# Don-Yin/VAE-GAN

Measured on NVIDIA B200. Metric: train_images_per_sec, higher is better.
Workload: dtype bf16

## Files before the change

### vae_gan_b200/csrc/conv_tc.cu

```cuda
#include <algorithm>
#include <array>
#include <map>
#include <mutex>
#include <vector>
#include "vg_common.cuh"
#include "sm100_ptx.cuh"

namespace vg {

struct TcTap {
  int8_t map, dy, dx, pad_;
  int32_t wrow;
};
struct TcPhase {
  int32_t ntaps, oy_off, ox_off, pad_;
  TcTap taps[16];
};
struct alignas(64) TcConvParams {
  CUtensorMap in_maps[4];
  CUtensorMap w_map;
  TcPhase phases[4];
  int tiles_x, tiles_y, tiles_n;
  int tw_log2, th_log2, TW, TH, TN;
  int gw, gh, gn;
  int k_chunks;
  int n_out;
  int n_store;
  int OH, OW, os;
  int out_f32;
  int ksplit, k_per_split;
  void* out;
  const float* bias;
  const float* colscale;
  const float* sigma;
  int sigma_group_n;
  float act_slope;
  const void* residual;
  void* out2;
  const float* post_scale;
  const float* post_shift;
  float post_slope;
  CUtensorMap out_maps[4];
  int tma_store;
  int* det_locks;
  long long det_split_stride;
};

struct alignas(64) TcWgradParams {
  CUtensorMap s_maps[4];
  CUtensorMap u_map;
  TcTap taps[16];
  int ntaps, cs_chunks, cs, cu;
  int tiles_x, tiles_y, tiles_n, TW, TH, TN;
  int n_boxes, boxes_per_split;
  int packed;
  float* dw;
  int* det_locks;
  long long det_split_stride;
};

constexpr int kTcThreads = 256;
constexpr int kABytes = 128 * 128;
constexpr int kStageBytes = 32 * 64;

template <int STAGES, int A_BYTES, int B_BYTES, int NACC, int EW>
struct TcSmem {
  static constexpr int kStages = STAGES, kA = A_BYTES, kB = B_BYTES;
  static constexpr int kBytes =
      1024 + STAGES * (A_BYTES + B_BYTES) + (2 * STAGES + NACC) * 8 + 16 + (EW > 0 ? 16 + 512 + EW * kStageBytes : 0);
  uint8_t* a;
  uint8_t* b;
  uint64_t* full;
  uint64_t* empty;
  uint64_t* acc;
  uint32_t* tmem_slot;
  uint8_t* stage;
  __device__ explicit TcSmem(uint8_t* raw) {
    a = raw + ((1024u - (ptx::smem_u32(raw) & 1023u)) & 1023u);
    b = a + STAGES * A_BYTES;
    full = reinterpret_cast<uint64_t*>(b + STAGES * B_BYTES);
    empty = full + STAGES;
    acc = empty + STAGES;
    tmem_slot = reinterpret_cast<uint32_t*>(acc + NACC);
    stage = reinterpret_cast<uint8_t*>((reinterpret_cast<uintptr_t>(tmem_slot + 4) + 511) & ~(uintptr_t)511);
  }
};

template <int BN, int STAGES>
using ConvSmem = TcSmem<STAGES, kABytes, BN * 128, 1, 4>;
template <int CTAS, int BN, int MT, int STAGES, int EW>
using ConvPersistSmem = TcSmem<STAGES, MT * kABytes, (BN / CTAS) * 128, 4, EW>;
template <int NB, int STAGES>
using WgradSmem = TcSmem<STAGES, (2 + NB) * 8192, 0, 1, 0>;

template <int CTAS, int TMEM_COLS, class Smem, class InitAcc>
__device__ __forceinline__ uint32_t tc_prologue(const Smem& sm, const CUtensorMap* map0, const CUtensorMap* map1, InitAcc init_acc) {
  const int warp = threadIdx.x >> 5, lane = threadIdx.x & 31;
  if (warp == 0 && lane == 0) {
    ptx::prefetch_tmap(map0);
    ptx::prefetch_tmap(map1);
  }
  if (warp == 1 && lane == 0) {
    for (int s = 0; s < Smem::kStages; ++s) {
      ptx::mbar_init(&sm.full[s], 1);
      ptx::mbar_init(&sm.empty[s], 1);
    }
    init_acc();
    ptx::fence_barrier_init();
  }
  if (warp == 2) {
    if constexpr (CTAS == 2) ptx::tmem_alloc_pair<TMEM_COLS>(sm.tmem_slot);
    else ptx::tmem_alloc<TMEM_COLS>(sm.tmem_slot);
  }
  ptx::tc_fence_before();
  if constexpr (CTAS == 2) ptx::cluster_sync();
  else __syncthreads();
  ptx::tc_fence_after();
  vg::pdl_entry();
  return *sm.tmem_slot;
}

template <int CTAS, int TMEM_COLS>
__device__ __forceinline__ void tc_teardown(uint32_t tmem_base) {
  ptx::tc_fence_before();
  if constexpr (CTAS == 2) ptx::cluster_sync();
  else __syncthreads();
  if ((threadIdx.x >> 5) == 2) {
    if constexpr (CTAS == 2) ptx::tmem_dealloc_pair<TMEM_COLS>(tmem_base);
    else ptx::tmem_dealloc<TMEM_COLS>(tmem_base);
  }
}

struct Tile { int x0, y0, n0; };
template <class P>
__device__ __forceinline__ Tile tile_origin(const P& p, int t) {
  const int tx = t % p.tiles_x; t /= p.tiles_x;
  const int ty = t % p.tiles_y;
  const int tn = t / p.tiles_y;
  return Tile{tx * p.TW, ty * p.TH, tn * p.TN};
}

template <class Smem>
struct RingPos {
  int stage = 0;
  uint32_t phase = 0;
  __device__ __forceinline__ bool next() {
    if (++stage < Smem::kStages) return false;
    stage = 0;
    phase ^= 1u;
    return true;
  }
};

template <bool INF>
__device__ __forceinline__ void epilogue_chunk(const TcConvParams& p, const uint32_t (&r)[32], bool valid, long long opix, int gn,
                                               int ncol, bool first_chunk, uint8_t* stage, int sx, int sy, int sn, int z) {
  const int lane = threadIdx.x & 31;
  const bool add_bias = p.ksplit <= 1 || z == 0;
  float v[32];
#pragma unroll
  for (int j = 0; j < 32; ++j) v[j] = __uint_as_float(r[j]);
  if (p.sigma != nullptr && valid) {
    const float inv = 1.0f / __ldg(p.sigma + (p.sigma_group_n > 0 ? gn / p.sigma_group_n : 0));
#pragma unroll
    for (int j = 0; j < 32; ++j) v[j] *= inv;
  }
  if (p.bias != nullptr && add_bias) {
#pragma unroll
    for (int j = 0; j < 32; ++j)
      if (ncol + j < p.n_out) v[j] += __ldg(p.bias + ncol + j);
  }
  if (p.colscale != nullptr && valid) {
    const float* cs = p.colscale + (long long)gn * p.n_out + ncol;
#pragma unroll
// ... 122 lines not shown
        }
        *reinterpret_cast<uint4*>(o + j) = make_uint4(w[0], w[1], w[2], w[3]);
      }
    }
  }
}


__device__ __forceinline__ const TcPhase& conv_slice(const TcConvParams& p, int z, int& kb0, int& kb1) {
  const TcPhase& ph = p.phases[p.ksplit > 1 ? 0 : z];
  const int total = ph.ntaps * p.k_chunks;
  if (p.ksplit > 1) { kb0 = z * p.k_per_split; kb1 = min(total, kb0 + p.k_per_split); }
  else { kb0 = 0; kb1 = total; }
  if (kb1 < kb0) kb1 = kb0;
  return ph;
}

template <int CTAS, int MT, class Smem>
__device__ __forceinline__ void load_item(const TcConvParams& p, const TcPhase& ph, int kb0, int kb1, const Tile (&t)[MT], int nvalid,
                                          int wrow0, uint32_t rank, const Smem& sm, RingPos<Smem>& pos) {
  int tp = kb0 / p.k_chunks, kc = kb0 % p.k_chunks;
  for (int i = kb0; i < kb1; ++i) {
    const TcTap tap = ph.taps[tp];
    const CUtensorMap* im = &p.in_maps[tap.map];
    ptx::mbar_wait(&sm.empty[pos.stage], pos.phase ^ 1u);
    if (ptx::elect_one()) {
      uint8_t* a = sm.a + pos.stage * Smem::kA;
      uint8_t* b = sm.b + pos.stage * Smem::kB;
      if constexpr (CTAS == 2) {
        if (rank == 0) ptx::mbar_arrive_expect_tx(&sm.full[pos.stage], 2 * (Smem::kA + Smem::kB));
        const uint32_t bar = ptx::mapa(ptx::smem_u32(&sm.full[pos.stage]), 0);
#pragma unroll
        for (int m = 0; m < MT; ++m)
          ptx::tma_load_4d_pair(a + m * kABytes, im, bar, kc * 64, t[m].x0 + tap.dx, t[m].y0 + tap.dy, t[m].n0);
        ptx::tma_load_2d_pair(b, &p.w_map, bar, kc * 64, tap.wrow + wrow0);
      } else {
        ptx::mbar_arrive_expect_tx(&sm.full[pos.stage], nvalid * kABytes + Smem::kB);
#pragma unroll
        for (int m = 0; m < MT; ++m)
          if (m < nvalid)
            ptx::tma_load_4d(a + m * kABytes, im, &sm.full[pos.stage], kc * 64, t[m].x0 + tap.dx, t[m].y0 + tap.dy, t[m].n0);
        ptx::tma_load_2d(b, &p.w_map, &sm.full[pos.stage], kc * 64, tap.wrow + wrow0);
      }
    }
    __syncwarp();
    pos.next();
    if (++kc == p.k_chunks) { kc = 0; ++tp; }
  }
}

template <int CTAS>
__device__ __forceinline__ void commit_to(uint64_t* bar) {
  if constexpr (CTAS == 2) ptx::mma_commit_pair(bar, 3);
  else ptx::mma_commit(bar);
}

template <int CTAS, int BN, int MT, class Smem>
__device__ __forceinline__ void mma_item(uint32_t acc, int num_k, int nvalid, const Smem& sm, RingPos<Smem>& pos, uint32_t a_lo0,
                                         uint32_t b_lo0, uint32_t& a_lo, uint32_t& b_lo) {
  constexpr uint32_t idesc = ptx::make_idesc_bf16(128 * CTAS, BN, 0, 0);
  constexpr uint32_t kDescHi = ptx::smem_desc_hi(1024);
  for (int i = 0; i < num_k; ++i) {
    ptx::mbar_wait(&sm.full[pos.stage], pos.phase);
    ptx::tc_fence_after();
    if (ptx::elect_one()) {
#pragma unroll
      for (int m = 0; m < MT; ++m) {
        if (m < nvalid) {
#pragma unroll
          for (int k = 0; k < 4; ++k) {
            const uint32_t d = acc + (uint32_t)(m * BN), a = a_lo + (uint32_t)((m * kABytes + k * 32) >> 4),
                           b = b_lo + (uint32_t)((k * 32) >> 4);
            if constexpr (CTAS == 2) ptx::mma_bf16_ss_pair_lohi(d, a, b, kDescHi, idesc, (i | k) != 0);
            else ptx::mma_bf16_ss_lohi(d, a, b, kDescHi, idesc, (i | k) != 0);
          }
        }
      }
      commit_to<CTAS>(&sm.empty[pos.stage]);
    }
    __syncwarp();
    if (pos.next()) { a_lo = a_lo0; b_lo = b_lo0; }
    else { a_lo += (uint32_t)(Smem::kA >> 4); b_lo += (uint32_t)(Smem::kB >> 4); }
  }
}

struct EpiWarp {
  int ew, q, cgrp;
  int xl, yl, nl;
  int xl0, yl0, nl0;
  __device__ explicit EpiWarp(const TcConvParams& p) {
    ew = (int)(threadIdx.x >> 5) - 4;
    q = ew & 3;
    cgrp = ew >> 2;
    const int row = q * 32 + (threadIdx.x & 31), row0 = q * 32;
    xl = row & (p.TW - 1);
    yl = (row >> p.tw_log2) & (p.TH - 1);
    nl = row >> (p.tw_log2 + p.th_log2);
    xl0 = row0 & (p.TW - 1), yl0 = (row0 >> p.tw_log2) & (p.TH - 1), nl0 = row0 >> (p.tw_log2 + p.th_log2);
  }
};

template <int BN, int EW, bool INF>
__device__ __forceinline__ void drain_tile(const TcConvParams& p, const TcPhase& ph, const EpiWarp& e, uint32_t acc, bool has_k, Tile t,
                                           bool live, int ncol0, int z, uint8_t* stage_base) {
  const int gx = t.x0 + e.xl, gy = t.y0 + e.yl, gn = t.n0 + e.nl;
  const bool valid = gx < p.gw && gy < p.gh && gn < p.gn && live;
  const long long opix = ((long long)gn * p.OH + (long long)gy * p.os + ph.oy_off) * p.OW + (long long)gx * p.os + ph.ox_off;
#pragma unroll(EW == 4 ? BN / 32 : 1)
  for (int i = 0; i < BN / EW / 8; ++i) {
    const int c = EW == 4 ? i : i * (EW / 4) + e.cgrp;
    const int c0 = c * 32;
    uint32_t r[32];
    if (has_k) {
      ptx::tmem_ld_32x32(acc + ((uint32_t)(e.q * 32) << 16) + (uint32_t)c0, r);
      ptx::tmem_ld_wait();
    } else {
#pragma unroll
      for (int j = 0; j < 32; ++j) r[j] = 0u;
    }
    epilogue_chunk<INF>(p, r, valid, opix, gn, ncol0 + c0, c == 0, stage_base + e.ew * kStageBytes, t.x0 + e.xl0, t.y0 + e.yl0,
                        t.n0 + e.nl0, z);
  }
}

template <int BN, int STAGES, bool INF>
__global__ void __launch_bounds__(kTcThreads) tc_conv_kernel(const __grid_constant__ TcConvParams p) {
  using Smem = ConvSmem<BN, STAGES>;
  extern __shared__ uint8_t smem_raw[];
  const Smem sm(smem_raw);
  uint64_t* const tmem_full = sm.acc;
  const int warp = threadIdx.x >> 5, lane = threadIdx.x & 31;
  const int z = (int)blockIdx.z;
  int kb0, kb1;
  const TcPhase& ph = conv_slice(p, z, kb0, kb1);
  const bool has_k = kb1 > kb0;
  const Tile t = tile_origin(p, (int)blockIdx.x);
  const int ncol0 = blockIdx.y * BN;
  const uint32_t tmem_base = tc_prologue<1, BN>(sm, &p.w_map, &p.in_maps[0], [&] { ptx::mbar_init(tmem_full, 1); });

  if (has_k) {
    RingPos<Smem> pos;
    if (warp == 0) {
      const Tile ts[1] = {t};
      load_item<1, 1>(p, ph, kb0, kb1, ts, 1, ncol0, 0, sm, pos);
    } else if (warp == 1) {
      const uint32_t a_lo0 = ptx::smem_desc_lo(ptx::smem_u32(sm.a), 16), b_lo0 = ptx::smem_desc_lo(ptx::smem_u32(sm.b), 16);
      uint32_t a_lo = a_lo0, b_lo = b_lo0;
      mma_item<1, BN, 1>(tmem_base, kb1 - kb0, 1, sm, pos, a_lo0, b_lo0, a_lo, b_lo);
      if (ptx::elect_one()) ptx::mma_commit(tmem_full);
      __syncwarp();
    }
  }

  if (warp >= 4) {
    if (has_k) {
      ptx::mbar_wait(tmem_full, 0);
      ptx::tc_fence_after();
    }
    int* const det_lock = (p.det_locks != nullptr && p.ksplit > 1) ? p.det_locks + (blockIdx.y * gridDim.x + blockIdx.x) : nullptr;
    if (det_lock) {
      if (lane == 0) det_wait_turn(det_lock, z);
      __syncwarp();
    }
    const bool live = !(p.ksplit > 1 && !has_k && p.det_split_stride == 0);
    drain_tile<BN, 4, INF>(p, ph, EpiWarp(p), tmem_base, has_k, t, live, ncol0, z, sm.stage);
    if (det_lock) {
      __threadfence();
      asm volatile("bar.sync 2, 128;" ::: "memory");
      if (warp == 4 && lane == 0) det_publish_turn(det_lock, z + 1 == p.ksplit ? 0 : z + 1);
    }
    if (!INF && p.tma_store && lane == 0) ptx::bulk_wait_group0();
  }
  tc_teardown<1, BN>(tmem_base);
}

template <int CTAS, int BN, int MT, int STAGES, int EW, bool INF>
__device__ __forceinline__ void conv_persistent(const TcConvParams& p, int n_ntiles, int n_groups, int n_work) {
  static_assert(EW == 4 || EW == 8, "4 or 8 epilogue warps");
  constexpr int kAccCols = MT * BN;
  constexpr int kTmemCols = 2 * kAccCols;
  static_assert(kTmemCols <= 512 && kTmemCols >= 32, "TMEM budget");
  using Smem = ConvPersistSmem<CTAS, BN, MT, STAGES, EW>;
  extern __shared__ uint8_t smem_raw[];
  const Smem sm(smem_raw);
  uint64_t* const acc_full = sm.acc;
  uint64_t* const acc_empty = sm.acc + 2;
  const int warp = threadIdx.x >> 5, lane = threadIdx.x & 31;
  const uint32_t rank = CTAS == 2 ? ptx::cluster_ctarank() : 0u;
  const int w_first = blockIdx.x / CTAS, w_step = gridDim.x / CTAS;
  const int total_tiles = p.tiles_x * p.tiles_y * p.tiles_n;
  const uint32_t tmem_base = tc_prologue<CTAS, kTmemCols>(sm, &p.w_map, &p.in_maps[0], [&] {
    for (int a = 0; a < 2; ++a) {
      ptx::mbar_init(&acc_full[a], 1);
      ptx::mbar_init(&acc_empty[a], CTAS * EW);
    }
  });

  auto decode = [&](int w, int& z, int& nt, int& g) {
    const int per_z = n_ntiles * n_groups;
    z = w / per_z;
    const int r = w - z * per_z;
    nt = r / n_groups;
    g = r - nt * n_groups;
  };
  auto tiles_of = [&](int g, int& tile0, int& nvalid) {
    tile0 = (g * CTAS + (int)rank) * MT;
    nvalid = CTAS == 2 ? MT : min(MT, total_tiles - tile0);
  };

  if (warp == 0) {
    RingPos<Smem> pos;
    for (int w = w_first; w < n_work; w += w_step) {
      int z, nt, g, kb0, kb1, tile0, nvalid;
      decode(w, z, nt, g);
      const TcPhase& ph = conv_slice(p, z, kb0, kb1);
      if (kb1 == kb0) continue;
      tiles_of(g, tile0, nvalid);
      Tile t[MT];
#pragma unroll
      for (int m = 0; m < MT; ++m) t[m] = tile_origin(p, tile0 + m);
      load_item<CTAS, MT>(p, ph, kb0, kb1, t, nvalid, nt * BN + (int)rank * (BN / CTAS), rank, sm, pos);
    }
  } else if (warp == 1) {
    if (rank == 0) {
      const uint32_t a_lo0 = ptx::smem_desc_lo(ptx::smem_u32(sm.a), 16), b_lo0 = ptx::smem_desc_lo(ptx::smem_u32(sm.b), 16);
      uint32_t a_lo = a_lo0, b_lo = b_lo0;
      RingPos<Smem> pos;
      int it = 0;
      for (int w = w_first; w < n_work; w += w_step) {
        int z, nt, g, kb0, kb1, tile0, nvalid;
        decode(w, z, nt, g);
        conv_slice(p, z, kb0, kb1);
        if (kb1 == kb0) continue;
        tiles_of(g, tile0, nvalid);
        const int as = it & 1;
        ptx::mbar_wait(&acc_empty[as], (uint32_t)(((it >> 1) & 1) ^ 1));
        ptx::tc_fence_after();
        mma_item<CTAS, BN, MT>(tmem_base + (uint32_t)(as * kAccCols), kb1 - kb0, nvalid, sm, pos, a_lo0, b_lo0, a_lo, b_lo);
        if (ptx::elect_one()) commit_to<CTAS>(&acc_full[as]);
        __syncwarp();
        ++it;
      }
    }
  } else if (warp >= 4) {
    const EpiWarp e(p);
    int it = 0;
    for (int w = w_first; w < n_work; w += w_step) {
      int z, nt, g, kb0, kb1, tile0, nvalid;
      decode(w, z, nt, g);
      const TcPhase& ph = conv_slice(p, z, kb0, kb1);
      const bool has_k = kb1 > kb0;
      if (!has_k && p.ksplit > 1) continue;
      tiles_of(g, tile0, nvalid);
      const int as = it & 1;
      if (has_k) {
        ptx::mbar_wait(&acc_full[as], (uint32_t)((it >> 1) & 1));
        ptx::tc_fence_after();
      }
#pragma unroll 1
      for (int m = 0; m < nvalid; ++m)
        drain_tile<BN, EW, INF>(p, ph, e, tmem_base + (uint32_t)(as * kAccCols + m * BN), has_k, tile_origin(p, tile0 + m), true, nt * BN,
                                z, sm.stage);
      if (has_k) {
        ptx::tc_fence_before();
        __syncwarp();
        if (lane == 0) {
          if constexpr (CTAS == 2) ptx::mbar_arrive_cluster(ptx::mapa(ptx::smem_u32(&acc_empty[as]), 0));
          else ptx::mbar_arrive(&acc_empty[as]);
        }
        ++it;
      }
    }
    if (!INF && p.tma_store && lane == 0) ptx::bulk_wait_group0();
  }
  tc_teardown<CTAS, kTmemCols>(tmem_base);
}

template <int BN, int MT, int STAGES, int EW, bool INF>
__global__ void __launch_bounds__(128 + 32 * EW, 1)
    tc_conv_persist_kernel(const __grid_constant__ TcConvParams p, int n_ntiles, int n_groups, int n_work) {
  conv_persistent<1, BN, MT, STAGES, EW, INF>(p, n_ntiles, n_groups, n_work);
}

template <int BN, int MT, int STAGES, int EW, bool INF>
__global__ void __cluster_dims__(2, 1, 1) __launch_bounds__(128 + 32 * EW, 1)
    tc_conv_pair_kernel(const __grid_constant__ TcConvParams p, int n_ntiles, int n_groups, int n_work) {
  conv_persistent<2, BN, MT, STAGES, EW, INF>(p, n_ntiles, n_groups, n_work);
}

template <int NB, int STAGES>
__global__ void __launch_bounds__(kTcThreads) tc_wgrad_kernel(const __grid_constant__ TcWgradParams p) {
  using Smem = WgradSmem<NB, STAGES>;
  extern __shared__ uint8_t smem_raw[];
  constexpr int BN = NB * 64;
  constexpr int kStageBytes = Smem::kA;
  const Smem sm(smem_raw);
  uint8_t* const smem = sm.a;
  uint64_t* const full = sm.full;
  uint64_t* const empty = sm.empty;
  uint64_t* const tmem_full = sm.acc;

  const int warp = threadIdx.x >> 5, lane = threadIdx.x & 31;
  const int n_slabs = p.ntaps * p.cs_chunks;
  const int slab0 = blockIdx.x * 2;
  const bool has2 = slab0 + 1 < n_slabs;
  const int slab1 = has2 ? slab0 + 1 : slab0;
  const int box_begin = blockIdx.z * p.boxes_per_split;
  const int box_end = min(p.n_boxes, box_begin + p.boxes_per_split);
  const int num_k = max(0, box_end - box_begin);

  const uint32_t tmem_base = tc_prologue<1, BN>(sm, &p.u_map, &p.s_maps[0], [&] { ptx::mbar_init(tmem_full, 1); });

  if (num_k > 0) {
    if (warp == 0) {
      const int tapA = slab0 / p.cs_chunks, chA = slab0 % p.cs_chunks;
      const int tapB = slab1 / p.cs_chunks, chB = slab1 % p.cs_chunks;
      const TcTap ta = p.taps[tapA], tb = p.taps[tapB];
      int stage = 0;
      uint32_t phase = 0;
      for (int b = box_begin; b < box_end; ++b) {
        const Tile t = tile_origin(p, b);
        const int x0 = t.x0, y0 = t.y0, n0 = t.n0;
        ptx::mbar_wait(&empty[stage], phase ^ 1u);
        if (ptx::elect_one()) {
          ptx::mbar_arrive_expect_tx(&full[stage], kStageBytes);
          uint8_t* st = smem + stage * kStageBytes;
          ptx::tma_load_4d(st, &p.s_maps[ta.map], &full[stage], chA * 64, x0 + ta.dx, y0 + ta.dy, n0);
          ptx::tma_load_4d(st + 8192, &p.s_maps[tb.map], &full[stage], chB * 64, x0 + tb.dx, y0 + tb.dy, n0);
#pragma unroll
          for (int j = 0; j < NB; ++j)
            ptx::tma_load_4d(st + (2 + j) * 8192, &p.u_map, &full[stage], (blockIdx.y * NB + j) * 64, x0, y0, n0);
        }
        __syncwarp();
        if (++stage == STAGES) { stage = 0; phase ^= 1u; }
      }
    } else if (warp == 1) {
      constexpr uint32_t idesc = ptx::make_idesc_bf16(128, BN, 1, 1);
      constexpr uint32_t kDescHi = ptx::smem_desc_hi(1024);
      const uint32_t a_lo0 = ptx::smem_desc_lo(ptx::smem_u32(smem), 8192);
      uint32_t a_lo = a_lo0;
      int stage = 0;
      uint32_t phase = 0;
      for (int i = 0; i < num_k; ++i) {
        ptx::mbar_wait(&full[stage], phase);
        ptx::tc_fence_after();
        if (ptx::elect_one()) {
#pragma unroll
          for (int k = 0; k < 4; ++k)
            ptx::mma_bf16_ss_lohi(tmem_base, a_lo + (uint32_t)((k * 2048) >> 4), a_lo + (uint32_t)((2 * 8192 + k * 2048) >> 4), kDescHi,
                                  idesc, (i | k) != 0);
          ptx::mma_commit(&empty[stage]);
        }
        __syncwarp();
        if (++stage == STAGES) { stage = 0; phase ^= 1u; a_lo = a_lo0; }
        else a_lo += (uint32_t)(kStageBytes >> 4);
      }
      if (ptx::elect_one()) ptx::mma_commit(tmem_full);
      __syncwarp();
    }
  }

  int* const det_lock = p.det_locks != nullptr ? p.det_locks + (blockIdx.y * gridDim.x + blockIdx.x) : nullptr;
  if (warp >= 4 && det_lock) {
    if (lane == 0) det_wait_turn(det_lock, (int)blockIdx.z);
    __syncwarp();
  }
  if (warp >= 4 && num_k > 0) {
    const int q = warp - 4;
    const int row = q * 32 + lane;
    const int slab = (row < 64) ? slab0 : slab1;
// ... 141 lines not shown
  int l = 0;
  while ((1 << l) < v) ++l;
  return l;
}

static void choose_box(int gw, int gh, int gn, int pixels, int* TW, int* TH, int* TN) {
  double best = 1e30;
  int bw = 1, bh = 1;
  for (int tw = 1; tw <= pixels; tw *= 2)
    for (int th = 1; tw * th <= pixels; th *= 2) {
      int tn = pixels / (tw * th);
      if (tw > 256 || th > 256 || tn > 256) continue;
      double padded = (double)cdiv(gw, tw) * tw * (double)cdiv(gh, th) * th * (double)cdiv(gn, tn) * tn;
      double score = padded - 1e-3 * tw - 1e-6 * th;
      if (score < best) { best = score; bw = tw; bh = th; }
    }
  *TW = bw; *TH = bh; *TN = pixels / (bw * bh);
}

static bool tc_common_supported(const VgConvDesc* d) {
  if (g_force_simt) return false;
  if (d->act_dtype != VG_BF16) return false;
  if (d->stride != 1 && d->stride != 2) return false;
  if (d->kh != d->kw || d->kh * d->kw > 16) return false;
  if (d->stride == 2 && ((d->transposed ? d->h_out : d->h_in) % 2 != 0 || (d->transposed ? d->w_out : d->w_in) % 2 != 0)) return false;
  return get_encode() != nullptr;
}

bool tc_conv_supported(const VgConvDesc* d, bool dgrad) {
  const int c_red = dgrad ? d->c_out : d->c_in;
  const int n_out = dgrad ? d->c_in : d->c_out;
  return c_red % 64 == 0 && (n_out % 64 == 0 || n_out == 1) && tc_common_supported(d);
}

bool tc_wgrad_supported(const VgConvDesc* d) {
  return d->c_in % 64 == 0 && d->c_out % 64 == 0 && tc_common_supported(d);
}

template <auto Kernel, class... Args>
static int launch(dim3 grid, int threads, int smem, cudaStream_t s, const Args&... args) {
  static std::once_flag once;
  static cudaError_t attr_err = cudaSuccess;
  std::call_once(once, [smem] { attr_err = cudaFuncSetAttribute(Kernel, cudaFuncAttributeMaxDynamicSharedMemorySize, smem); });
  VG_CUDA(attr_err);
  vg::Launch(grid, threads, smem, s)(Kernel, args...);
  VG_LAUNCHED();
  return VG_OK;
}

static void build_gather_taps(TcPhase* ph, int k, int stride, int pad, int n_out) {
  ph->ntaps = 0; ph->oy_off = 0; ph->ox_off = 0;
  for (int ky = 0; ky < k; ++ky)
    for (int kx = 0; kx < k; ++kx) {
      TcTap& t = ph->taps[ph->ntaps++];
      const int ty = ky - pad, tx = kx - pad;
      if (stride == 1) {
        t.map = 0; t.dy = (int8_t)ty; t.dx = (int8_t)tx;
      } else {
        const int py = ((ty % 2) + 2) % 2, px = ((tx % 2) + 2) % 2;
        t.map = (int8_t)(py * 2 + px);
        t.dy = (int8_t)((ty - py) / 2);
        t.dx = (int8_t)((tx - px) / 2);
      }
      t.pad_ = 0;
      t.wrow = (ky * k + kx) * n_out;
    }
}
static void build_scatter_phase(TcPhase* ph, int k, int stride, int pad, int n_out, int phy, int phx) {
  ph->ntaps = 0; ph->oy_off = phy; ph->ox_off = phx;
  for (int ky = 0; ky < k; ++ky) {
    if (((phy + pad - ky) % stride + stride) % stride != 0) continue;
    for (int kx = 0; kx < k; ++kx) {
      if (((phx + pad - kx) % stride + stride) % stride != 0) continue;
      TcTap& t = ph->taps[ph->ntaps++];
      t.map = 0;
      t.dy = (int8_t)((phy + pad - ky) / stride);
      t.dx = (int8_t)((phx + pad - kx) / stride);
      t.pad_ = 0;
      t.wrow = (ky * k + kx) * n_out;
    }
  }
}

enum TuneForm { kFormAuto = 0, kFormOneShot = 1, kFormPersist = 2, kFormPair = 3 };
using TuneKey = std::array<int, 10>;
struct TuneVal { int bn, form; };
static std::map<TuneKey, TuneVal> g_tune;
static std::vector<TuneKey> g_tune_seen;
static bool g_tune_record = false;
static std::mutex g_tune_mu;
static TuneKey tune_key(const VgConvDesc* d, bool dgrad) {
  return TuneKey{dgrad ? 1 : 0, d->n, d->h_in, d->w_in, d->c_in, d->c_out, d->kh, d->stride, d->pad, d->transposed ? 1 : 0};
}
static TuneVal tune_lookup(const VgConvDesc* d, bool dgrad) {
  std::lock_guard<std::mutex> lk(g_tune_mu);
  const TuneKey k = tune_key(d, dgrad);
  if (g_tune_record && std::find(g_tune_seen.begin(), g_tune_seen.end(), k) == g_tune_seen.end()) g_tune_seen.push_back(k);
  auto it = g_tune.find(k);
  return it == g_tune.end() ? TuneVal{0, kFormAuto} : it->second;
}
int tc_tune_set(const VgConvDesc* d, int dgrad, int bn, int form) {
  VG_CHECK_ARG(d != nullptr, "null descriptor");
  VG_CHECK_ARG(bn == 0 || bn == 64 || bn == 128 || bn == 256, "N tile must be 0 (heuristic), 64, 128 or 256 (got %d)", bn);
  VG_CHECK_ARG(form >= kFormAuto && form <= kFormPair, "kernel form must be 0..3 (got %d)", form);
  std::lock_guard<std::mutex> lk(g_tune_mu);
  if (bn == 0 && form == kFormAuto) g_tune.erase(tune_key(d, dgrad != 0));
  else g_tune[tune_key(d, dgrad != 0)] = TuneVal{bn, form};
  return VG_OK;
}
void tc_tune_clear() {
  std::lock_guard<std::mutex> lk(g_tune_mu);
  g_tune.clear();
}
void tc_tune_record(int on) {
  std::lock_guard<std::mutex> lk(g_tune_mu);
  g_tune_record = on != 0;
  if (on) g_tune_seen.clear();
}
int tc_tune_seen(int* keys, int max_keys) {
  std::lock_guard<std::mutex> lk(g_tune_mu);
  const int n = (int)std::min<size_t>(g_tune_seen.size(), (size_t)std::max(0, max_keys));
  for (int i = 0; i < n && keys != nullptr; ++i)
    for (int j = 0; j < 10; ++j) keys[i * 10 + j] = g_tune_seen[i][j];
  return (int)g_tune_seen.size();
}

static int pick_bn(int n_out) {
  if (n_out % 256 == 0) return 256;
  if (n_out % 128 == 0) return 128;
  return 64;
}

constexpr int kPersistMinItemsPerSm64 = 6;
constexpr int kPairMinBN = 128;

template <int CTAS, int BN, int MT, int STAGES, int EW, bool INF>
static int launch_persistent(const TcConvParams& p, dim3 grid, cudaStream_t s) {
  const int n_groups = (int)cdiv(grid.x, CTAS * MT);
  const int n_work = (int)((long long)n_groups * grid.y * grid.z);
  const int ctas = CTAS * std::min(n_work, num_sms() / CTAS);
  const int threads = 128 + 32 * EW, smem = ConvPersistSmem<CTAS, BN, MT, STAGES, EW>::kBytes;
  if constexpr (CTAS == 2)
    return launch<tc_conv_pair_kernel<BN, MT, STAGES, EW, INF>>(ctas, threads, smem, s, p, (int)grid.y, n_groups, n_work);
  else
    return launch<tc_conv_persist_kernel<BN, MT, STAGES, EW, INF>>(ctas, threads, smem, s, p, (int)grid.y, n_groups, n_work);
}

template <bool INF>
static int launch_conv(int form, int BN, const TcConvParams& p, dim3 grid, cudaStream_t s) {
  switch (form * 1000 + BN) {
    case kFormOneShot * 1000 + 64: return launch<tc_conv_kernel<64, 4, INF>>(grid, kTcThreads, ConvSmem<64, 4>::kBytes, s, p);
    case kFormOneShot * 1000 + 128: return launch<tc_conv_kernel<128, 3, INF>>(grid, kTcThreads, ConvSmem<128, 3>::kBytes, s, p);
    case kFormOneShot * 1000 + 256: return launch<tc_conv_kernel<256, 4, INF>>(grid, kTcThreads, ConvSmem<256, 4>::kBytes, s, p);
    case kFormPersist * 1000 + 64: return launch_persistent<1, 64, 4, 3, 4, INF>(p, grid, s);
    case kFormPersist * 1000 + 128: return launch_persistent<1, 128, 2, 4, 8, INF>(p, grid, s);
    case kFormPersist * 1000 + 256: return launch_persistent<1, 256, 1, 4, 8, INF>(p, grid, s);
    case kFormPair * 1000 + 64: return launch_persistent<2, 64, 4, 3, 4, INF>(p, grid, s);
    case kFormPair * 1000 + 128: return launch_persistent<2, 128, 2, 4, 8, INF>(p, grid, s);
    case kFormPair * 1000 + 256: return launch_persistent<2, 256, 1, 6, 8, INF>(p, grid, s);
    default: set_error("unsupported BN %d", BN); return VG_EUNSUPPORTED;
  }
}

int tc_conv_run(const VgConvDesc* d, bool dgrad, const void* in, const void* wpack, const float* bias, const float* colscale,
                const float* sigma, int sigma_group_n, void* out, int out_dtype, cudaStream_t s, const VgConvEpilogue* ep) {
  TcConvParams p;
  memset(&p, 0, sizeof(p));
  const bool gather = (d->transposed != 0) == dgrad;
  const int in_h = dgrad ? d->h_out : d->h_in, in_w = dgrad ? d->w_out : d->w_in, in_c = dgrad ? d->c_out : d->c_in;
  const int out_h = dgrad ? d->h_in : d->h_out, out_w = dgrad ? d->w_in : d->w_out, n_out = dgrad ? d->c_in : d->c_out;
  const int k = d->kh, st = d->stride, pad = d->pad;
  p.k_chunks = in_c / 64;
  p.n_out = n_out;
  p.OH = out_h; p.OW = out_w;
  p.out = out; p.out_f32 = out_dtype == VG_F32;
  p.bias = bias; p.colscale = colscale;
  p.sigma = sigma; p.sigma_group_n = sigma_group_n;
  p.act_slope = 1.0f; p.post_slope = 1.0f;
  if (ep != nullptr) {
    p.act_slope = ep->act_slope; p.residual = ep->residual; p.out2 = ep->y2;
    p.post_scale = ep->post_scale; p.post_shift = ep->post_shift; p.post_slope = ep->post_slope;
  }
  int nphase = 1;
  if (gather) {
    p.gw = out_w; p.gh = out_h; p.gn = d->n; p.os = 1;
    build_gather_taps(&p.phases[0], k, st, pad, n_out);
  } else {
    p.os = st;
    nphase = st * st;
    p.gw = (out_w + st - 1) / st; p.gh = (out_h + st - 1) / st; p.gn = d->n;
    for (int phy = 0; phy < st; ++phy)
      for (int phx = 0; phx < st; ++phx) build_scatter_phase(&p.phases[phy * st + phx], k, st, pad, n_out, phy, phx);
  }
  choose_box(p.gw, p.gh, p.gn, 128, &p.TW, &p.TH, &p.TN);
  p.tw_log2 = ilog2(p.TW); p.th_log2 = ilog2(p.TH);
  p.tiles_x = (int)cdiv(p.gw, p.TW); p.tiles_y = (int)cdiv(p.gh, p.TH); p.tiles_n = (int)cdiv(p.gn, p.TN);
  int rc;
  if (gather && st == 2) {
    for (int py = 0; py < 2; ++py)
      for (int px = 0; px < 2; ++px)
        if ((rc = make_act_map(&p.in_maps[py * 2 + px], in, d->n, in_h, in_w, in_c, 2, py, px, p.TW, p.TH, p.TN))) return rc;
  } else {
    if ((rc = make_act_map(&p.in_maps[0], in, d->n, in_h, in_w, in_c, 1, 0, 0, p.TW, p.TH, p.TN))) return rc;
    p.in_maps[1] = p.in_maps[2] = p.in_maps[3] = p.in_maps[0];
  }
  const TuneVal tuned = tune_lookup(d, dgrad);
  const int BN = (n_out == 1) ? 64 : ((tuned.bn != 0 && n_out % tuned.bn == 0) ? tuned.bn : pick_bn(n_out));
  p.n_store = (n_out == 1) ? 1 : BN;
  if ((rc = make_weight_map(&p.w_map, wpack, (long long)k * k * n_out, in_c, BN))) return rc;
  dim3 grid((unsigned)(p.tiles_x * p.tiles_y * p.tiles_n), (unsigned)std::max(1, n_out / BN), (unsigned)nphase);
  if (grid.x == 0) return VG_OK;
  if (ep != nullptr && (ep->act_slope != 1.0f || ep->residual != nullptr || ep->y2 != nullptr) && (p.out_f32 || p.n_store == 1)) {
    set_error("the activation / residual / second-output epilogue needs a bf16 output with c_out %% 64 == 0");
    return VG_EUNSUPPORTED;
  }
  p.ksplit = 1;
  p.k_per_split = p.phases[0].ntaps * p.k_chunks;
  {
    const long long ctas = (long long)grid.x * grid.y;
    const int total_kb = p.phases[0].ntaps * p.k_chunks;
    if (nphase == 1 && p.out_f32 && colscale == nullptr && ctas * 2 <= num_sms() && total_kb >= 16) {
      int ks = (int)std::min<long long>(cdiv(2LL * num_sms(), ctas), total_kb / 4);
      if (ks > 1) {
        p.k_per_split = (int)cdiv(total_kb, ks);
        p.ksplit = (int)cdiv(total_kb, p.k_per_split);
        grid.z = (unsigned)p.ksplit;
        const size_t out_elems = (size_t)d->n * out_h * out_w * n_out;
        VG_CUDA(cudaMemsetAsync(out, 0, out_elems * sizeof(float), s));
        if (g_det.on) {
          if ((size_t)p.ksplit * out_elems * sizeof(float) <= g_det.scratch_bytes) {
            p.out = g_det.scratch;
            p.det_split_stride = (long long)out_elems;
          } else if (!(p.det_locks = det_locks(ctas))) {
            return VG_EINVAL;
          }
        }
      }
    }
  }
  static int tma_store = -1;
  if (tma_store < 0) { const char* e = getenv("VG_TC_TMA_STORE"); tma_store = e ? atoi(e) : 2; }
  if (tma_store && !p.out_f32 && p.ksplit == 1 && p.n_store != 1 && (p.os == 1 || tma_store >= 2) &&
      p.act_slope == 1.0f && p.residual == nullptr && p.out2 == nullptr) {
    const int bx = std::min(p.TW, 32), by = std::min(p.TH, 32 / bx), bn = 32 / (bx * by);
    for (int ph = 0; ph < nphase; ++ph)
      if ((rc = make_out_map(&p.out_maps[ph], out, d->n, out_h, out_w, n_out, bx, by, bn, p.os, p.phases[ph].oy_off, p.phases[ph].ox_off)))
        return rc;
    p.tma_store = 1;
  }
  const long long ctas1 = (long long)grid.x * grid.y * grid.z;
  const bool heur_persist = !(g_det.on && p.ksplit > 1) &&
                            ((BN == 256 && ctas1 > (long long)num_sms()) ||
                             (BN == 128 && ctas1 >= 2LL * num_sms()) ||
                             (BN == 64 && ctas1 >= (long long)kPersistMinItemsPerSm64 * num_sms()));
  const int form = p.ksplit > 1 ? kFormAuto : tuned.form;
  const bool use_persist = form == kFormAuto ? heur_persist : (form != kFormOneShot);
  int run_form = use_persist ? kFormPersist : kFormOneShot;
  if (use_persist && p.n_store != 1 && (form == kFormPair || (form == kFormAuto && BN >= kPairMinBN))) {
    const int mt = BN == 64 ? 4 : (BN == 128 ? 2 : 1);
    if (grid.x % (2 * mt) == 0) {
      if ((rc = make_weight_map(&p.w_map, wpack, (long long)k * k * n_out, in_c, BN / 2))) return rc;
      run_form = kFormPair;
    }
  }
  const bool inf = p.act_slope != 1.0f || p.residual != nullptr || p.out2 != nullptr;
  rc = inf ? launch_conv<true>(run_form, BN, p, grid, s) : launch_conv<false>(run_form, BN, p, grid, s);
  if (rc == VG_OK && p.det_split_stride != 0)
    rc = ordered_reduce_f32((const float*)p.out, p.ksplit, p.det_split_stride, (float*)out, s);
  return rc;
}

int tc_wgrad_run(const VgConvDesc* d, const void* x, const void* dy, float* dw, float* workspace, cudaStream_t s, bool acc_only) {
  TcWgradParams p;
  memset(&p, 0, sizeof(p));
  const void *U, *S;
  int hu, wu, cu, hs, ws, cs;
  if (!d->transposed) { U = dy; hu = d->h_out; wu = d->w_out; cu = d->c_out; S = x; hs = d->h_in; ws = d->w_in; cs = d->c_in; }
  else                { U = x;  hu = d->h_in;  wu = d->w_in;  cu = d->c_in;  S = dy; hs = d->h_out; ws = d->w_out; cs = d->c_out; }
  const int k = d->kh, st = d->stride, pad = d->pad;
  TcPhase tmp;
  build_gather_taps(&tmp, k, st, pad, 0);
  p.ntaps = tmp.ntaps;
  for (int i = 0; i < tmp.ntaps; ++i) p.taps[i] = tmp.taps[i];
  p.cs_chunks = cs / 64; p.cs = cs; p.cu = cu;
  choose_box(wu, hu, d->n, 64, &p.TW, &p.TH, &p.TN);
  p.tiles_x = (int)cdiv(wu, p.TW); p.tiles_y = (int)cdiv(hu, p.TH); p.tiles_n = (int)cdiv(d->n, p.TN);
  p.n_boxes = p.tiles_x * p.tiles_y * p.tiles_n;
  p.packed = workspace != nullptr && tmp.ntaps > 1;
  p.dw = (p.packed || acc_only) ? workspace : dw;
  const size_t welems = (size_t)k * k * cs * cu;
  if (p.packed && !acc_only) VG_CUDA(cudaMemsetAsync(workspace, 0, welems * sizeof(float), s));
  int rc;
  if (st == 2) {
    for (int py = 0; py < 2; ++py)
      for (int px = 0; px < 2; ++px)
        if ((rc = make_act_map(&p.s_maps[py * 2 + px], S, d->n, hs, ws, cs, 2, py, px, p.TW, p.TH, p.TN))) return rc;
  } else {
    if ((rc = make_act_map(&p.s_maps[0], S, d->n, hs, ws, cs, 1, 0, 0, p.TW, p.TH, p.TN))) return rc;
    p.s_maps[1] = p.s_maps[2] = p.s_maps[3] = p.s_maps[0];
  }
  if ((rc = make_act_map(&p.u_map, U, d->n, hu, wu, cu, 1, 0, 0, p.TW, p.TH, p.TN))) return rc;
  const int NB = (cu % 256 == 0) ? 4 : ((cu % 128 == 0) ? 2 : 1);
  const int m_tiles = (p.ntaps * p.cs_chunks + 1) / 2;
  const int n_tiles = cu / (NB * 64);
  if (p.n_boxes == 0) return VG_OK;
  const long long tiles = (long long)m_tiles * n_tiles;
  long long splits = 1;
  {
    double best = -1.0;
    const long long max_splits = std::max<long long>(1, p.n_boxes / 4);
    for (long long waves = 1; waves <= 4; ++waves) {
      long long sp = std::max<long long>(1, std::min<long long>((waves * num_sms()) / tiles, max_splits));
      long long bps = cdiv(p.n_boxes, sp);
      sp = cdiv(p.n_boxes, bps);
      const long long ctas = tiles * sp;
      const double eff = (double)ctas / (double)(cdiv(ctas, num_sms()) * num_sms());
      const double score = eff - 0.02 * (double)sp / (double)max_splits - (ctas < num_sms() ? 0.5 : 0.0);
      if (score > best) { best = score; splits = sp; }
    }
  }
  p.boxes_per_split = (int)cdiv(p.n_boxes, splits);
  splits = cdiv(p.n_boxes, p.boxes_per_split);
  dim3 grid((unsigned)m_tiles, (unsigned)n_tiles, (unsigned)splits);
  float* const wgrad_dst = p.dw;
  if (g_det.on && splits > 1) {
    if ((size_t)splits * welems * sizeof(float) <= g_det.scratch_bytes) {
      p.dw = (float*)g_det.scratch;
      p.det_split_stride = (long long)welems;
    } else if (!(p.det_locks = det_locks(tiles))) {
      return VG_EINVAL;
    }
  }
  switch (NB) {
    case 1: rc = launch<tc_wgrad_kernel<1, 6>>(grid, kTcThreads, WgradSmem<1, 6>::kBytes, s, p); break;
    case 2: rc = launch<tc_wgrad_kernel<2, 5>>(grid, kTcThreads, WgradSmem<2, 5>::kBytes, s, p); break;
    default: rc = launch<tc_wgrad_kernel<4, 4>>(grid, kTcThreads, WgradSmem<4, 4>::kBytes, s, p); break;
  }
  if (rc == VG_OK && p.det_split_stride != 0) rc = ordered_reduce_f32(p.dw, (int)splits, p.det_split_stride, wgrad_dst, s);
  if (rc || !p.packed || acc_only) return rc;
  dim3 ug((unsigned)cdiv((long long)cs * p.ntaps, 32), (unsigned)cdiv(cu, 32));
  vg::Launch(ug, 256, 0, s)(wgrad_unpack_kernel, workspace, cu, cs, p.ntaps, dw);
  VG_LAUNCHED();
  return VG_OK;
}

}
// ... 1 lines not shown
```

### vae_gan_b200/tune.py

```python
from __future__ import annotations

import ctypes as C
import json
import os
from pathlib import Path
from typing import Callable, Dict, List, Tuple

import torch

from . import _lib

Key = Tuple[int, ...]
FORMS = {0: "heuristic", 1: "one-shot", 2: "persistent", 3: "cta-pair"}
DEFAULT_TABLE = Path(__file__).resolve().parent / "tile_table.json"


def _desc(key: Key) -> _lib.VgConvDesc:
    dgrad, n, h, w, cin, cout, k, stride, pad, tr = key
    if tr:
        ho, wo = (h - 1) * stride - 2 * pad + k, (w - 1) * stride - 2 * pad + k
    else:
        ho, wo = (h + 2 * pad - k) // stride + 1, (w + 2 * pad - k) // stride + 1
    return _lib.VgConvDesc(n, h, w, cin, ho, wo, cout, k, k, stride, pad, tr, _lib.VG_BF16, _lib.VG_BF16)


def set_entry(key: Key, bn: int, form: int):
    _lib.call("vg_conv_tune_set", C.byref(_desc(key)), int(key[0]), int(bn), int(form))


def clear():
    _lib.call("vg_conv_tune_clear")


def record(fn: Callable[[], None]) -> List[Key]:
    _lib.call("vg_conv_tune_record", 1)
    try:
        fn()
        torch.cuda.synchronize()
    finally:
        _lib.call("vg_conv_tune_record", 0)
    cnt = C.c_int(0)
    _lib.call("vg_conv_tune_seen", None, 0, C.byref(cnt))
    buf = (C.c_int * (10 * max(1, cnt.value)))()
    _lib.call("vg_conv_tune_seen", C.cast(buf, C.c_void_p), cnt.value, C.byref(cnt))
    return [tuple(buf[i * 10 + j] for j in range(10)) for i in range(cnt.value)]


def _time_key(key: Key, iters: int) -> float:
    dgrad, n, h, w, cin, cout, k, stride, pad, tr = key
    dev = torch.device("cuda", torch.cuda.current_device())
    d = _desc(key)
    g = torch.Generator(device=dev).manual_seed(0)
    x = torch.randn(n, h, w, cin, generator=g, device=dev, dtype=torch.bfloat16)
    y = torch.empty(n, d.h_out, d.w_out, cout, device=dev, dtype=torch.bfloat16)
    wt = torch.randn(k * k * cin * cout, generator=g, device=dev) / (cin * k * k) ** 0.5
    pk = torch.empty(wt.numel(), dtype=torch.bfloat16, device=dev)
    pn = torch.empty_like(pk)
    s = _lib.stream_ptr()
    _lib.call("vg_conv_pack_weights", C.byref(d), wt.data_ptr(), None, pk.data_ptr(), pn.data_ptr(), s)
    if dgrad:
        dy = torch.randn(y.shape, generator=g, device=dev, dtype=torch.bfloat16)
        dx = torch.empty_like(x)
        run = lambda: _lib.call("vg_conv_dgrad", C.byref(d), dy.data_ptr(), pk.data_ptr(), pn.data_ptr(), dx.data_ptr(), s)
    else:
        run = lambda: _lib.call("vg_conv_forward", C.byref(d), x.data_ptr(), pk.data_ptr(), pn.data_ptr(), None, None, y.data_ptr(), None, s)
    for _ in range(3):
        run()
    torch.cuda.synchronize()
    evs = [(torch.cuda.Event(enable_timing=True), torch.cuda.Event(enable_timing=True)) for _ in range(iters)]
    for a, b in evs:
        a.record()
        run()
        b.record()
    torch.cuda.synchronize()
    ts = sorted(a.elapsed_time(b) for a, b in evs)
    return ts[len(ts) // 2]


def autotune(fn: Callable[[], None] = None, keys: List[Key] = None, iters: int = 15, min_gain: float = 0.03, verbose: bool = False) -> Dict[Key, dict]:
    if keys is None:
        keys = record(fn)
    table: Dict[Key, dict] = {}
    for key in keys:
        dgrad, n, h, w, cin, cout, k, stride, pad, tr = key
        n_out = cin if dgrad else cout
        if n_out % 64 != 0 or (h == 1 and w == 1):
            continue
        set_entry(key, 0, 0)
        base = _time_key(key, iters)
        best = (base, 0, 0)
        for bn in (64, 128, 256):
            if n_out % bn != 0:
                continue
            for form in (1, 2, 3):
                set_entry(key, bn, form)
                try:
# ... 42 lines not shown
```

Baseline: 4392.

## Add column conv form with SMEM-resident weights and halo-reused activation boxes

Adds a persistent 'column' kernel form for 3x3 stride-1 convs with 64 channels in and out. All nine tap weights are loaded into shared memory once per CTA. Each work item loads three halo-extended activation boxes (one per dx), and the nine taps are addressed as offsets into those boxes. This replaces re-fetching weights and shifted activations for every tap with a single halo load per tile. It is picked automatically when the shape matches, and it uses more shared memory and only two pipeline stages.

```diff
diff --git a/vae_gan_b200/csrc/conv_tc.cu b/vae_gan_b200/csrc/conv_tc.cu
--- a/vae_gan_b200/csrc/conv_tc.cu
+++ b/vae_gan_b200/csrc/conv_tc.cu
@@ -1,6 +1,7 @@
 #include <algorithm>
 #include <array>
 #include <map>
+#include <type_traits>
 #include <mutex>
 #include <vector>
 #include "vg_common.cuh"
@@ -63,11 +64,12 @@
 constexpr int kABytes = 128 * 128;
 constexpr int kStageBytes = 32 * 64;
 
-template <int STAGES, int A_BYTES, int B_BYTES, int NACC, int EW>
+template <int STAGES, int A_BYTES, int B_BYTES, int NACC, int EW, int W_BYTES = 0>
 struct TcSmem {
   static constexpr int kStages = STAGES, kA = A_BYTES, kB = B_BYTES;
-  static constexpr int kBytes =
-      1024 + STAGES * (A_BYTES + B_BYTES) + (2 * STAGES + NACC) * 8 + 16 + (EW > 0 ? 16 + 512 + EW * kStageBytes : 0);
+  static constexpr int kBytes = 1024 + W_BYTES + STAGES * (A_BYTES + B_BYTES) + (2 * STAGES + NACC) * 8 + 16 +
+                                (EW > 0 ? 16 + 512 + EW * kStageBytes : 0);
+  uint8_t* w;
   uint8_t* a;
   uint8_t* b;
   uint64_t* full;
@@ -76,7 +78,8 @@
   uint32_t* tmem_slot;
   uint8_t* stage;
   __device__ explicit TcSmem(uint8_t* raw) {
-    a = raw + ((1024u - (ptx::smem_u32(raw) & 1023u)) & 1023u);
+    w = raw + ((1024u - (ptx::smem_u32(raw) & 1023u)) & 1023u);
+    a = w + W_BYTES;
     b = a + STAGES * A_BYTES;
     full = reinterpret_cast<uint64_t*>(b + STAGES * B_BYTES);
     empty = full + STAGES;
@@ -90,6 +93,9 @@
 using ConvSmem = TcSmem<STAGES, kABytes, BN * 128, 1, 4>;
 template <int CTAS, int BN, int MT, int STAGES, int EW>
 using ConvPersistSmem = TcSmem<STAGES, MT * kABytes, (BN / CTAS) * 128, 4, EW>;
+constexpr int kColBoxBytes = kABytes + 2 * 32 * 128;
+template <int STAGES, int EW>
+using ColumnSmem = TcSmem<STAGES, 3 * kColBoxBytes, 0, 5, EW, 9 * 64 * 128>;
 template <int NB, int STAGES>
 using WgradSmem = TcSmem<STAGES, (2 + NB) * 8192, 0, 1, 0>;
 
@@ -378,6 +384,66 @@
     if (pos.next()) { a_lo = a_lo0; b_lo = b_lo0; }
     else { a_lo += (uint32_t)(Smem::kA >> 4); b_lo += (uint32_t)(Smem::kB >> 4); }
   }
+}
+
+struct ColumnTaps {
+  int dx0, dy0;
+  uint32_t a_off[9];
+  __device__ ColumnTaps(const TcConvParams& p, const TcPhase& ph) {
+    dx0 = dy0 = 127;
+#pragma unroll
+    for (int t = 0; t < 9; ++t) { dx0 = min(dx0, (int)ph.taps[t].dx); dy0 = min(dy0, (int)ph.taps[t].dy); }
+#pragma unroll
+    for (int t = 0; t < 9; ++t)
+      a_off[t] = (uint32_t)(((ph.taps[t].dx - dx0) * kColBoxBytes + (ph.taps[t].dy - dy0) * p.TW * 128) >> 4);
+  }
+};
+
+template <class Smem>
+__device__ __forceinline__ void load_column_weights(const TcConvParams& p, const TcPhase& ph, const Smem& sm, uint64_t* wbar) {
+  if (ptx::elect_one()) {
+    ptx::mbar_arrive_expect_tx(wbar, 9 * 64 * 128);
+#pragma unroll
+    for (int t = 0; t < 9; ++t) ptx::tma_load_2d(sm.w + t * 64 * 128, &p.w_map, wbar, 0, ph.taps[t].wrow);
+  }
+  __syncwarp();
+}
+
+template <class Smem>
+__device__ __forceinline__ void load_column_item(const TcConvParams& p, const ColumnTaps& ct, Tile t, const Smem& sm,
+                                                 RingPos<Smem>& pos) {
+  ptx::mbar_wait(&sm.empty[pos.stage], pos.phase ^ 1u);
+  if (ptx::elect_one()) {
+    uint8_t* a = sm.a + pos.stage * Smem::kA;
+    ptx::mbar_arrive_expect_tx(&sm.full[pos.stage], (uint32_t)(3 * (p.TH + 2) * p.TW * 128));
+#pragma unroll
+    for (int j = 0; j < 3; ++j)
+      ptx::tma_load_4d(a + j * kColBoxBytes, &p.in_maps[0], &sm.full[pos.stage], 0, t.x0 + ct.dx0 + j, t.y0 + ct.dy0, t.n0);
+  }
+  __syncwarp();
+  pos.next();
+}
+
+template <int BN, class Smem>
+__device__ __forceinline__ void mma_column_item(uint32_t acc, const ColumnTaps& ct, const Smem& sm, RingPos<Smem>& pos,
+                                                uint32_t a_lo0, uint32_t& a_lo, uint32_t w_lo) {
+  constexpr uint32_t idesc = ptx::make_idesc_bf16(128, BN, 0, 0);
+  constexpr uint32_t kDescHi = ptx::smem_desc_hi(1024);
+  ptx::mbar_wait(&sm.full[pos.stage], pos.phase);
+  ptx::tc_fence_after();
+  if (ptx::elect_one()) {
+#pragma unroll
+    for (int t = 0; t < 9; ++t) {
+#pragma unroll
+      for (int k = 0; k < 4; ++k)
+        ptx::mma_bf16_ss_lohi(acc, a_lo + ct.a_off[t] + (uint32_t)((k * 32) >> 4), w_lo + (uint32_t)((t * 64 * 128 + k * 32) >> 4),
+                              kDescHi, idesc, (t | k) != 0);
+    }
+    ptx::mma_commit(&sm.empty[pos.stage]);
+  }
+  __syncwarp();
+  if (pos.next()) a_lo = a_lo0;
+  else a_lo += (uint32_t)(Smem::kA >> 4);
 }
 
 struct EpiWarp {
@@ -470,13 +536,14 @@
   tc_teardown<1, BN>(tmem_base);
 }
 
-template <int CTAS, int BN, int MT, int STAGES, int EW, bool INF>
+template <int CTAS, int BN, int MT, int STAGES, int EW, bool INF, bool COLUMN = false>
 __device__ __forceinline__ void conv_persistent(const TcConvParams& p, int n_ntiles, int n_groups, int n_work) {
   static_assert(EW == 4 || EW == 8, "4 or 8 epilogue warps");
+  static_assert(!COLUMN || (CTAS == 1 && MT == 1 && BN == 64), "column form: single CTAs, one 64-wide pixel tile per item");
   constexpr int kAccCols = MT * BN;
   constexpr int kTmemCols = 2 * kAccCols;
   static_assert(kTmemCols <= 512 && kTmemCols >= 32, "TMEM budget");
-  using Smem = ConvPersistSmem<CTAS, BN, MT, STAGES, EW>;
+  using Smem = std::conditional_t<COLUMN, ColumnSmem<STAGES, EW>, ConvPersistSmem<CTAS, BN, MT, STAGES, EW>>;
   extern __shared__ uint8_t smem_raw[];
   const Smem sm(smem_raw);
   uint64_t* const acc_full = sm.acc;
@@ -490,6 +557,7 @@
       ptx::mbar_init(&acc_full[a], 1);
       ptx::mbar_init(&acc_empty[a], CTAS * EW);
     }
+    if constexpr (COLUMN) ptx::mbar_init(&sm.acc[4], 1);
   });
 
   auto decode = [&](int w, int& z, int& nt, int& g) {
@@ -504,7 +572,28 @@
     nvalid = CTAS == 2 ? MT : min(MT, total_tiles - tile0);
   };
 
-  if (warp == 0) {
+  if constexpr (COLUMN) {
+    const ColumnTaps ct(p, p.phases[0]);
+    if (warp == 0) {
+      load_column_weights(p, p.phases[0], sm, &sm.acc[4]);
+      RingPos<Smem> pos;
+      for (int w = w_first; w < n_work; w += w_step) load_column_item(p, ct, tile_origin(p, w), sm, pos);
+    } else if (warp == 1) {
+      const uint32_t a_lo0 = ptx::smem_desc_lo(ptx::smem_u32(sm.a), 16), w_lo = ptx::smem_desc_lo(ptx::smem_u32(sm.w), 16);
+      uint32_t a_lo = a_lo0;
+      RingPos<Smem> pos;
+      ptx::mbar_wait(&sm.acc[4], 0);
+      int it = 0;
+      for (int w = w_first; w < n_work; w += w_step, ++it) {
+        const int as = it & 1;
+        ptx::mbar_wait(&acc_empty[as], (uint32_t)(((it >> 1) & 1) ^ 1));
+        ptx::tc_fence_after();
+        mma_column_item<BN>(tmem_base + (uint32_t)(as * kAccCols), ct, sm, pos, a_lo0, a_lo, w_lo);
+        if (ptx::elect_one()) ptx::mma_commit(&acc_full[as]);
+        __syncwarp();
+      }
+    }
+  } else if (warp == 0) {
     RingPos<Smem> pos;
     for (int w = w_first; w < n_work; w += w_step) {
       int z, nt, g, kb0, kb1, tile0, nvalid;
@@ -538,7 +627,8 @@
         ++it;
       }
     }
-  } else if (warp >= 4) {
+  }
+  if (warp >= 4) {
     const EpiWarp e(p);
     int it = 0;
     for (int w = w_first; w < n_work; w += w_step) {
@@ -582,6 +672,12 @@
 __global__ void __cluster_dims__(2, 1, 1) __launch_bounds__(128 + 32 * EW, 1)
     tc_conv_pair_kernel(const __grid_constant__ TcConvParams p, int n_ntiles, int n_groups, int n_work) {
   conv_persistent<2, BN, MT, STAGES, EW, INF>(p, n_ntiles, n_groups, n_work);
+}
+
+template <int BN, int MT, int STAGES, int EW, bool INF>
+__global__ void __launch_bounds__(128 + 32 * EW, 1)
+    tc_conv_column_kernel(const __grid_constant__ TcConvParams p, int n_ntiles, int n_groups, int n_work) {
+  conv_persistent<1, BN, MT, STAGES, EW, INF, true>(p, n_ntiles, n_groups, n_work);
 }
 
 template <int NB, int STAGES>
@@ -889,7 +985,7 @@
   }
 }
 
-enum TuneForm { kFormAuto = 0, kFormOneShot = 1, kFormPersist = 2, kFormPair = 3 };
+enum TuneForm { kFormAuto = 0, kFormOneShot = 1, kFormPersist = 2, kFormPair = 3, kFormColumn = 4 };
 using TuneKey = std::array<int, 10>;
 struct TuneVal { int bn, form; };
 static std::map<TuneKey, TuneVal> g_tune;
@@ -909,7 +1005,7 @@
 int tc_tune_set(const VgConvDesc* d, int dgrad, int bn, int form) {
   VG_CHECK_ARG(d != nullptr, "null descriptor");
   VG_CHECK_ARG(bn == 0 || bn == 64 || bn == 128 || bn == 256, "N tile must be 0 (heuristic), 64, 128 or 256 (got %d)", bn);
-  VG_CHECK_ARG(form >= kFormAuto && form <= kFormPair, "kernel form must be 0..3 (got %d)", form);
+  VG_CHECK_ARG(form >= kFormAuto && form <= kFormColumn, "kernel form must be 0..4 (got %d)", form);
   std::lock_guard<std::mutex> lk(g_tune_mu);
   if (bn == 0 && form == kFormAuto) g_tune.erase(tune_key(d, dgrad != 0));
   else g_tune[tune_key(d, dgrad != 0)] = TuneVal{bn, form};
@@ -941,13 +1037,16 @@
 constexpr int kPersistMinItemsPerSm64 = 6;
 constexpr int kPairMinBN = 128;
 
-template <int CTAS, int BN, int MT, int STAGES, int EW, bool INF>
+template <int CTAS, int BN, int MT, int STAGES, int EW, bool INF, bool COLUMN = false>
 static int launch_persistent(const TcConvParams& p, dim3 grid, cudaStream_t s) {
   const int n_groups = (int)cdiv(grid.x, CTAS * MT);
   const int n_work = (int)((long long)n_groups * grid.y * grid.z);
   const int ctas = CTAS * std::min(n_work, num_sms() / CTAS);
-  const int threads = 128 + 32 * EW, smem = ConvPersistSmem<CTAS, BN, MT, STAGES, EW>::kBytes;
-  if constexpr (CTAS == 2)
+  const int threads = 128 + 32 * EW;
+  const int smem = COLUMN ? ColumnSmem<STAGES, EW>::kBytes : ConvPersistSmem<CTAS, BN, MT, STAGES, EW>::kBytes;
+  if constexpr (COLUMN)
+    return launch<tc_conv_column_kernel<BN, MT, STAGES, EW, INF>>(ctas, threads, smem, s, p, (int)grid.y, n_groups, n_work);
+  else if constexpr (CTAS == 2)
     return launch<tc_conv_pair_kernel<BN, MT, STAGES, EW, INF>>(ctas, threads, smem, s, p, (int)grid.y, n_groups, n_work);
   else
     return launch<tc_conv_persist_kernel<BN, MT, STAGES, EW, INF>>(ctas, threads, smem, s, p, (int)grid.y, n_groups, n_work);
@@ -965,6 +1064,7 @@
     case kFormPair * 1000 + 64: return launch_persistent<2, 64, 4, 3, 4, INF>(p, grid, s);
     case kFormPair * 1000 + 128: return launch_persistent<2, 128, 2, 4, 8, INF>(p, grid, s);
     case kFormPair * 1000 + 256: return launch_persistent<2, 256, 1, 6, 8, INF>(p, grid, s);
+    case kFormColumn * 1000 + 64: return launch_persistent<1, 64, 1, 2, 4, INF, true>(p, grid, s);
     default: set_error("unsupported BN %d", BN); return VG_EUNSUPPORTED;
   }
 }
@@ -1069,6 +1169,11 @@
       if ((rc = make_weight_map(&p.w_map, wpack, (long long)k * k * n_out, in_c, BN / 2))) return rc;
       run_form = kFormPair;
     }
+  }
+  if (use_persist && BN == 64 && (form == kFormColumn || form == kFormAuto) && k == 3 && st == 1 && p.ksplit == 1 &&
+      p.k_chunks == 1 && n_out == 64 && p.TN == 1 && p.TW % 8 == 0 && p.TW <= 32) {
+    if ((rc = make_act_map(&p.in_maps[0], in, d->n, in_h, in_w, in_c, 1, 0, 0, p.TW, p.TH + 2, 1))) return rc;
+    run_form = kFormColumn;
   }
   const bool inf = p.act_slope != 1.0f || p.residual != nullptr || p.out2 != nullptr;
   rc = inf ? launch_conv<true>(run_form, BN, p, grid, s) : launch_conv<false>(run_form, BN, p, grid, s);
diff --git a/vae_gan_b200/tune.py b/vae_gan_b200/tune.py
--- a/vae_gan_b200/tune.py
+++ b/vae_gan_b200/tune.py
@@ -11,7 +11,7 @@
 from . import _lib
 
 Key = Tuple[int, ...]
-FORMS = {0: "heuristic", 1: "one-shot", 2: "persistent", 3: "cta-pair"}
+FORMS = {0: "heuristic", 1: "one-shot", 2: "persistent", 3: "cta-pair", 4: "column"}
 DEFAULT_TABLE = Path(__file__).resolve().parent / "tile_table.json"
 
 
```

New measurement: 4400, median of 6. About the same (+0.2%).
